# ufal/neuralmonkey

Measured on NVIDIA H100. Metric: train_target_tokens_per_sec, higher is better.
Workload: dtype f32 storage; tensor-core products in fp16 (vocabulary) / tf32 with fp32 accumulation

## Files before the change

neuralmonkey_b200/csrc/gru_cluster.cuh:

```cuda
#pragma once
#include "common.cuh"

namespace nm {

constexpr int GC_CLUSTER = 8;
constexpr int GC_SLICES = 32;
constexpr int GC_UPW = 4;
constexpr int GC_WARPS = 10;
constexpr int GC_THREADS = GC_WARPS * 32;
constexpr int GC_MAX_UNITS = GC_WARPS * GC_UPW;
constexpr int GC_RB = 2;
constexpr int GC_MAX_SL = 10;
constexpr int GC_SMEM_CAP = 200 * 1024;
constexpr int GC_BAR_BYTES = 64;
constexpr int GC_XS = 4;
constexpr int GC_PF = 8;

__host__ __device__ constexpr int gc_row(int SL) { return GC_SLICES * 4 * (((SL + 3) / 4) | 1); }
__host__ __device__ constexpr int gc_fwd_row_floats(int SL) {
  return 3 * gc_row(SL) + GC_MAX_UNITS * (1 + 2 * GC_XS) + 1;
}
__host__ __device__ constexpr int gc_bwd_row_floats(int SL) {
  return 4 * gc_row(SL) + GC_MAX_UNITS * (1 + 2 * GC_PF) + 1;
}

template <int SL>
struct GcGeom {
  static constexpr int SLP = 4 * (((SL + 3) / 4) | 1);
  static constexpr int ROW = GC_SLICES * SLP;
  static __device__ __forceinline__ int pos(int j) { return (j / SL) * SLP + (j % SL); }
};

__device__ __forceinline__ void cluster_barrier() {
  asm volatile("barrier.cluster.arrive.release.aligned;\n\tbarrier.cluster.wait.acquire.aligned;" ::
                   : "memory");
}
__device__ __forceinline__ uint32_t cluster_rank() {
  uint32_t r;
  asm volatile("mov.u32 %0, %%cluster_ctarank;" : "=r"(r));
  return r;
}

__device__ __forceinline__ uint32_t gc_smem_u32(const void* p) {
  return (uint32_t)__cvta_generic_to_shared(p);
}
__device__ __forceinline__ void gc_mbar_init(uint32_t bar) {
  asm volatile("mbarrier.init.shared::cta.b64 [%0], 1;" ::"r"(bar));
  asm volatile("fence.mbarrier_init.release.cluster;" ::: "memory");
}
__device__ __forceinline__ void gc_mbar_arm(uint32_t bar, uint32_t bytes) {
  asm volatile("mbarrier.arrive.expect_tx.shared::cta.b64 _, [%0], %1;" ::"r"(bar), "r"(bytes) : "memory");
}
__device__ __forceinline__ void gc_mbar_wait(uint32_t bar, uint32_t parity) {
  uint32_t done;
  do {
    asm volatile(
        "{\n\t.reg .pred p;\n\t"
        "mbarrier.try_wait.parity.acquire.cluster.shared::cta.b64 p, [%1], %2;\n\t"
        "selp.u32 %0, 1, 0, p;\n\t}"
        : "=r"(done)
        : "r"(bar), "r"(parity)
        : "memory");
  } while (!done);
}
__device__ __forceinline__ void gc_send(uint32_t addr, uint32_t bar, uint32_t dst, float v) {
  uint32_t ra, rb;
  asm volatile("mapa.shared::cluster.u32 %0, %1, %2;" : "=r"(ra) : "r"(addr), "r"(dst));
  asm volatile("mapa.shared::cluster.u32 %0, %1, %2;" : "=r"(rb) : "r"(bar), "r"(dst));
  asm volatile("st.async.shared::cluster.mbarrier::complete_tx::bytes.b32 [%0], %1, [%2];" ::"r"(ra),
               "r"(__float_as_uint(v)), "r"(rb)
               : "memory");
}

__device__ __forceinline__ void cp_async4(float* smem_dst, const float* gmem_src) {
  const uint32_t d = gc_smem_u32(smem_dst);
  asm volatile("cp.async.ca.shared.global [%0], [%1], 4;" ::"r"(d), "l"(gmem_src) : "memory");
}
__device__ __forceinline__ void cp_async_commit() { asm volatile("cp.async.commit_group;" ::: "memory"); }
__device__ __forceinline__ void cp_async_wait_all() { asm volatile("cp.async.wait_all;" ::: "memory"); }

template <int N, int O>
__device__ __forceinline__ void gc_reduce_level(float (&v)[N], int lane) {
  constexpr int n = N * O / 16;
  if constexpr (n > 1) {
    const bool upper = (lane & O) != 0;
#pragma unroll
    for (int i = 0; i < n / 2; ++i) {
      const float keep = upper ? v[i + n / 2] : v[i];
      const float send = upper ? v[i] : v[i + n / 2];
      v[i] = keep + __shfl_xor_sync(0xffffffffu, send, O);
    }
  } else {
    v[0] += __shfl_xor_sync(0xffffffffu, v[0], O);
  }
  if constexpr (O > 1) gc_reduce_level<N, O / 2>(v, lane);
}
template <int N>
__device__ __forceinline__ void gc_reduce_scatter(float (&v)[N], int lane) {
  gc_reduce_level<N, 16>(v, lane);
}

template <int SL>
__device__ __forceinline__ void gc_dot(const float* __restrict__ vec, int row0, int lane,
                                       const float (&w)[GC_UPW][SL], float (&acc)[GC_RB][GC_UPW]) {
#pragma unroll
  for (int r = 0; r < GC_RB; ++r)
#pragma unroll
    for (int u = 0; u < GC_UPW; ++u) acc[r][u] = 0.f;
  const float* base = vec + row0 * GcGeom<SL>::ROW + lane * GcGeom<SL>::SLP;
#pragma unroll
  for (int c = 0; c < SL; c += 4) {
    const int n = SL - c < 4 ? SL - c : 4;
#pragma unroll
    for (int r = 0; r < GC_RB; ++r) {
      const float* p = base + r * GcGeom<SL>::ROW + c;
      float x[4];
      if (n == 4) {
        const float4 q = *reinterpret_cast<const float4*>(p);
        x[0] = q.x; x[1] = q.y; x[2] = q.z; x[3] = q.w;
      } else {
        if (n >= 2) {
          const float2 q = *reinterpret_cast<const float2*>(p);
          x[0] = q.x; x[1] = q.y;
        }
        if (n == 1) x[0] = p[0];
        if (n == 3) x[2] = p[2];
      }
#pragma unroll
      for (int u = 0; u < GC_UPW; ++u)
#pragma unroll
        for (int i = 0; i < 4; ++i)
          if (i < n) acc[r][u] = fmaf(x[i], w[u][c + i], acc[r][u]);
    }
  }
}

template <int SL>
__device__ __forceinline__ void gc_load_w(float (&w)[GC_UPW][SL], const float* __restrict__ W,
                                          int64_t sk, int64_t su, int unit0, int unit_limit, int k0, int H) {
#pragma unroll
  for (int u = 0; u < GC_UPW; ++u)
#pragma unroll
    for (int i = 0; i < SL; ++i) {
      const int unit = unit0 + u, k = k0 + i;
      const bool ok = (unit < unit_limit) && (k < H);
      w[u][i] = ok ? W[(int64_t)k * sk + (int64_t)unit * su] : 0.f;
    }
}

struct GcProf {
  bool on;
  unsigned t0;
  __device__ __forceinline__ explicit GcProf(const long long* out)
      : on(out != nullptr && blockIdx.x == 0 && threadIdx.x == 0), t0(on ? (unsigned)clock() : 0u) {}
  __device__ __forceinline__ void lap(long long* out, int slot) {
    if (on) {
      const unsigned t1 = (unsigned)clock();
      out[slot] += (long long)(t1 - t0);
      t0 = t1;
    }
  }
};

struct GcFwdArgs {
  const float* xproj;
  const float* Wgh;
  const float* Wch;
  const float* h0;
  const int32_t* lengths;
  const float* drop_mask;
  float* states;
  float* raw_states;
  float* final_state;
  float* gates;
  float* hprev;
  float* rh;
  int B, T, H, Bc, reverse;
  long long* prof;
};

__device__ __forceinline__ void gc_fwd_prefetch(const GcFwdArgs& a, int t, float* dst, int b0, int nrows,
                                                int ubeg, int UW) {
  const int H = a.H, T = a.T;
  for (int idx = threadIdx.x; idx < a.Bc * UW; idx += GC_THREADS) {
    const int b = idx / UW, ul = idx - b * UW, j = ubeg + ul;
    if (b < nrows && j < H) {
      const int64_t row = ((int64_t)(b0 + b) * T + t);
      const float* xp = a.xproj + row * 3 * H + j;
      float* xd = dst + (b * GC_MAX_UNITS + ul) * GC_XS;
      cp_async4(xd, xp);
      cp_async4(xd + 1, xp + H);
      cp_async4(xd + 2, xp + 2 * H);
      if (a.drop_mask) cp_async4(xd + 3, a.drop_mask + row * H + j);
    }
  }
  cp_async_commit();
}

__device__ __forceinline__ uint32_t gc_phase_bytes(const GcFwdArgs& a) { return (uint32_t)(a.Bc * a.H * 4); }

template <int SL>
__global__ void __launch_bounds__(GC_THREADS, 1) gru_seq_fwd_cluster_kernel(GcFwdArgs a) {
  extern __shared__ __align__(16) float gc_smem[];
  constexpr int ROW = GcGeom<SL>::ROW;
  const int H = a.H, T = a.T, Bc = a.Bc;
  float* hbuf = gc_smem + GC_BAR_BYTES / 4;
  float* rhbuf = hbuf + 2 * Bc * ROW;
  float* us = rhbuf + Bc * ROW;
  float* xs = us + Bc * GC_MAX_UNITS;
  int* lens = reinterpret_cast<int*>(xs + 2 * Bc * GC_MAX_UNITS * GC_XS);
  const uint32_t bar_h = gc_smem_u32(gc_smem), bar_rh = bar_h + 16;

  const int rank = (int)cluster_rank();
  const int ubeg = rank * H / GC_CLUSTER;
  const int unit_limit = (rank + 1) * H / GC_CLUSTER;
  const int UW = unit_limit - ubeg;
  const int b0 = (blockIdx.x / GC_CLUSTER) * Bc;
  const int nrows = min(Bc, a.B - b0);
  const int lane = threadIdx.x & 31, warp = threadIdx.x >> 5;
  const int unit0_local = warp * GC_UPW;
  const int unit0 = ubeg + unit0_local;
  const bool warp_live = unit0 < unit_limit;

  float wr[GC_UPW][SL], wu[GC_UPW][SL], wc[GC_UPW][SL];
  gc_load_w<SL>(wr, a.Wgh, 2 * H, 1, unit0, unit_limit, lane * SL, H);
  gc_load_w<SL>(wu, a.Wgh + H, 2 * H, 1, unit0, unit_limit, lane * SL, H);
  gc_load_w<SL>(wc, a.Wch, H, 1, unit0, unit_limit, lane * SL, H);

  const int g1 = lane >> 4, r1 = (lane >> 3) & 1, u1 = (lane >> 1) & 3;
  const int r2 = (lane >> 4) & 1, u2 = (lane >> 2) & 3, copy2 = lane & 3;
  const int copy1 = ((lane >> 4) << 1) | (lane & 1);
  const bool ok1 = unit0 + u1 < unit_limit, ok2 = unit0 + u2 < unit_limit;
  const int j1 = unit0 + u1, j2 = unit0 + u2;
  const int pos1 = ok1 ? GcGeom<SL>::pos(j1) : 0, pos2 = ok2 ? GcGeom<SL>::pos(j2) : 0;

  if (threadIdx.x == 0) {
    gc_mbar_init(bar_h);
    gc_mbar_init(bar_h + 8);
    gc_mbar_init(bar_rh);
    gc_mbar_arm(bar_h, gc_phase_bytes(a));
    gc_mbar_arm(bar_h + 8, gc_phase_bytes(a));
    gc_mbar_arm(bar_rh, gc_phase_bytes(a));
  }
  for (int i = threadIdx.x; i < 3 * Bc * ROW; i += GC_THREADS) hbuf[i] = 0.f;
  for (int i = threadIdx.x; i < 2 * Bc * GC_MAX_UNITS * GC_XS; i += GC_THREADS) xs[i] = 0.f;
  for (int b = threadIdx.x; b < Bc; b += GC_THREADS)
    lens[b] = b < nrows ? (a.lengths ? a.lengths[b0 + b] : T) : 0;


  __syncthreads();
  cluster_barrier();
  const int t_first = a.reverse ? T - 1 : 0;
  for (int idx = threadIdx.x; idx < Bc * UW; idx += GC_THREADS) {
    const int b = idx / UW, j = ubeg + (idx - b * UW);
    const float hv = (b < nrows && a.h0) ? a.h0[(int64_t)(b0 + b) * H + j] : 0.f;
    if (b < nrows) a.hprev[((int64_t)(b0 + b) * T + t_first) * H + j] = hv;
    const uint32_t addr = gc_smem_u32(hbuf + b * ROW + GcGeom<SL>::pos(j));
    for (int d = 0; d < GC_CLUSTER; ++d) gc_send(addr, bar_h, d, hv);
  }
  gc_fwd_prefetch(a, t_first, xs, b0, nrows, ubeg, UW);

  GcProf prof(a.prof);
  for (int step = 0; step < T; ++step) {
    const int t = a.reverse ? T - 1 - step : step;
    const bool last = (step == T - 1);
    const int t_next = a.reverse ? t - 1 : t + 1;
    const int64_t row0 = (int64_t)b0 * T + t;
    const int par = step & 1;
    const float* hb = hbuf + par * Bc * ROW;
    const float* xc = xs + par * Bc * GC_MAX_UNITS * GC_XS;

    gc_mbar_wait(bar_h + 8 * par, (step >> 1) & 1);
    if (threadIdx.x == 0 && step + 2 < T) gc_mbar_arm(bar_h + 8 * par, gc_phase_bytes(a));
    prof.lap(a.prof, 0);
    cp_async_wait_all();
    __syncthreads();
    if (!last) gc_fwd_prefetch(a, t_next, xs + (par ^ 1) * Bc * GC_MAX_UNITS * GC_XS, b0, nrows, ubeg, UW);
    prof.lap(a.prof, 1);

    if (warp_live) {
      for (int r0 = 0; r0 < Bc; r0 += GC_RB) {
        float ar[GC_RB][GC_UPW], au[GC_RB][GC_UPW];
        gc_dot<SL>(hb, r0, lane, wr, ar);
        gc_dot<SL>(hb, r0, lane, wu, au);
        float v[2 * GC_RB * GC_UPW];
#pragma unroll
        for (int r = 0; r < GC_RB; ++r)
#pragma unroll
          for (int u = 0; u < GC_UPW; ++u) {
            v[r * GC_UPW + u] = ar[r][u];
            v[GC_RB * GC_UPW + r * GC_UPW + u] = au[r][u];
          }
        gc_reduce_scatter<2 * GC_RB * GC_UPW>(v, lane);
        const int b = r0 + r1, ul = unit0_local + u1;
        const float g = sigmoidf_(v[0] + xc[(b * GC_MAX_UNITS + ul) * GC_XS + g1]);
        const float rhv = g * hb[b * ROW + pos1];
        const float rh_peer = __shfl_xor_sync(0xffffffffu, rhv, 16);
        const float rh_send = g1 == 0 ? rhv : rh_peer;
        if (ok1) {
          if ((lane & 1) == 0) {
            if (b < nrows) {
              const int64_t row = row0 + (int64_t)b * T;
              a.gates[row * 3 * H + g1 * H + j1] = g;
              if (g1 == 0) a.rh[row * H + j1] = rhv;
            }
            if (g1 == 1) us[b * GC_MAX_UNITS + ul] = g;
          }
          const uint32_t addr = gc_smem_u32(rhbuf + b * ROW + pos1);
          gc_send(addr, bar_rh, 2 * copy1, rh_send);
          gc_send(addr, bar_rh, 2 * copy1 + 1, rh_send);
        }
      }
      __syncwarp();
    }
    prof.lap(a.prof, 2);
    gc_mbar_wait(bar_rh, step & 1);
    if (threadIdx.x == 0 && !last) gc_mbar_arm(bar_rh, gc_phase_bytes(a));
    prof.lap(a.prof, 3);

    if (warp_live) {
      const uint32_t bar_next = bar_h + 8 * (par ^ 1);
      float* hn_buf = hbuf + (par ^ 1) * Bc * ROW;
      for (int r0 = 0; r0 < Bc; r0 += GC_RB) {
        float ac[GC_RB][GC_UPW];
        gc_dot<SL>(rhbuf, r0, lane, wc, ac);
        float v[GC_RB * GC_UPW];
#pragma unroll
        for (int r = 0; r < GC_RB; ++r)
#pragma unroll
          for (int u = 0; u < GC_UPW; ++u) v[r * GC_UPW + u] = ac[r][u];
        gc_reduce_scatter<GC_RB * GC_UPW>(v, lane);
        if (!ok2) continue;
        const int b = r0 + r2, ul = unit0_local + u2;
        const float* xd = xc + (b * GC_MAX_UNITS + ul) * GC_XS;
        const float c = tanhf(v[0] + xd[2]);
        const float hv = hb[b * ROW + pos2];
        const float uu = us[b * GC_MAX_UNITS + ul];
        const bool live = t < lens[b];
        float hn = live ? (uu * hv + (1.f - uu) * c) : hv;
        const float raw = live ? hn : 0.f;
        if (a.drop_mask && live) hn *= xd[3];
        if (b < nrows) {
          const int64_t row = row0 + (int64_t)b * T;
          if (copy2 == 0) a.gates[row * 3 * H + 2 * H + j2] = c;
          else if (copy2 == 1) a.states[row * H + j2] = live ? hn : 0.f;
          else if (copy2 == 2) { if (a.raw_states) a.raw_states[row * H + j2] = raw; }
          else if (last) a.final_state[(int64_t)(b0 + b) * H + j2] = hn;
          else a.hprev[((int64_t)(b0 + b) * T + t_next) * H + j2] = hn;
        }
        if (!last) {
          const uint32_t addr = gc_smem_u32(hn_buf + b * ROW + pos2);
          gc_send(addr, bar_next, 2 * copy2, hn);
          gc_send(addr, bar_next, 2 * copy2 + 1, hn);
        }
      }
    }
    prof.lap(a.prof, 4);
  }
  cluster_barrier();
}

struct GcBwdArgs {
  const float* Wgh;
  const float* Wch;
  const int32_t* lengths;
  const float* drop_mask;
  const float* gates;
  const float* hprev;
  const float* dstates;
  const float* draw;
  const float* dfinal;
  float* dxproj;
  float* dh0;
  int B, T, H, Bc, reverse;
  long long* prof;
};

__device__ __forceinline__ float gc_bwd_e1(const GcBwdArgs& a, const float* pf, float dh, bool live,
                                           float& zc, float& zu) {
  if (!live) {
    zc = zu = 0.f;
    return dh;
  }
  const float uu = pf[1], c = pf[2], hv = pf[3];
  if (a.dstates) dh += pf[4];
  if (a.drop_mask) dh *= pf[5];
  if (a.draw) dh += pf[6];
  const float du = dh * (hv - c);
  const float dc = dh * (1.f - uu);
  zc = dc * (1.f - c * c);
  zu = du * uu * (1.f - uu);
  return dh * uu;
}

__device__ __forceinline__ void gc_bwd_prefetch(const GcBwdArgs& a, int t, float* dst, const int* lens, int b0,
                                                int ubeg, int UW) {
  const int H = a.H, T = a.T;
  for (int idx = threadIdx.x; idx < a.Bc * UW; idx += GC_THREADS) {
    const int b = idx / UW, u = idx - b * UW, j = ubeg + u;
    if (t >= lens[b]) continue;
    const int64_t row = (int64_t)(b0 + b) * T + t;
    float* d = dst + (b * GC_MAX_UNITS + u) * GC_PF;
    const float* g = a.gates + row * 3 * H + j;
    cp_async4(d, g);
    cp_async4(d + 1, g + H);
    cp_async4(d + 2, g + 2 * H);
    cp_async4(d + 3, a.hprev + row * H + j);
    if (a.dstates) cp_async4(d + 4, a.dstates + row * H + j);
    if (a.drop_mask) cp_async4(d + 5, a.drop_mask + row * H + j);
    if (a.draw) cp_async4(d + 6, a.draw + row * H + j);
  }
  cp_async_commit();
}

template <int SL>
__global__ void __launch_bounds__(GC_THREADS, 1) gru_seq_bwd_cluster_kernel(GcBwdArgs a) {
  extern __shared__ __align__(16) float gc_smem[];
  constexpr int ROW = GcGeom<SL>::ROW;
  const int H = a.H, T = a.T, Bc = a.Bc;
  float* vc = gc_smem + GC_BAR_BYTES / 4;
  float* vu = vc + Bc * ROW;
  float* vr = vu + 2 * Bc * ROW;
  float* dhp = vr + Bc * ROW;
  float* pf = dhp + Bc * GC_MAX_UNITS;
  int* lens = reinterpret_cast<int*>(pf + 2 * Bc * GC_MAX_UNITS * GC_PF);
  const uint32_t bar_a = gc_smem_u32(gc_smem), bar_b = bar_a + 16;
  const uint32_t bytes_a = (uint32_t)(2 * Bc * H * 4), bytes_b = (uint32_t)(Bc * H * 4);

  const int rank = (int)cluster_rank();
  const int ubeg = rank * H / GC_CLUSTER;
  const int unit_limit = (rank + 1) * H / GC_CLUSTER;
  const int UW = unit_limit - ubeg;
  const int b0 = (blockIdx.x / GC_CLUSTER) * Bc;
  const int nrows = min(Bc, a.B - b0);
  const int lane = threadIdx.x & 31, warp = threadIdx.x >> 5;
  const int unit0_local = warp * GC_UPW;
  const int unit0 = ubeg + unit0_local;
  const bool warp_live = unit0 < unit_limit;

  float w1[GC_UPW][SL], w2r[GC_UPW][SL], w2u[GC_UPW][SL];
  gc_load_w<SL>(w1, a.Wch, 1, H, unit0, unit_limit, lane * SL, H);
  gc_load_w<SL>(w2r, a.Wgh, 1, 2 * H, unit0, unit_limit, lane * SL, H);
  gc_load_w<SL>(w2u, a.Wgh + H, 1, 2 * H, unit0, unit_limit, lane * SL, H);

  const int rr_ = (lane >> 4) & 1, uq = (lane >> 2) & 3, copy = lane & 3;
  const bool ok = unit0 + uq < unit_limit;
  const int ji = unit0 + uq, ul = unit0_local + uq;
  const int pos = ok ? GcGeom<SL>::pos(ji) : 0;
  auto time_of = [reverse = a.reverse, T](int k) { return reverse ? k : T - 1 - k; };

  if (threadIdx.x == 0) {
    gc_mbar_init(bar_a);
    gc_mbar_init(bar_a + 8);
    gc_mbar_init(bar_b);
    gc_mbar_arm(bar_a, bytes_a);
    gc_mbar_arm(bar_a + 8, bytes_a);
    gc_mbar_arm(bar_b, bytes_b);
  }
  for (int i = threadIdx.x; i < 4 * Bc * ROW; i += GC_THREADS) vc[i] = 0.f;
  for (int i = threadIdx.x; i < 2 * Bc * GC_MAX_UNITS * GC_PF; i += GC_THREADS) pf[i] = 0.f;
  for (int b = threadIdx.x; b < Bc; b += GC_THREADS)
    lens[b] = b < nrows ? (a.lengths ? a.lengths[b0 + b] : T) : 0;
  __syncthreads();


  gc_bwd_prefetch(a, time_of(0), pf, lens, b0, ubeg, UW);
  cp_async_wait_all();
  __syncthreads();
  cluster_barrier();
  {
    const int t = time_of(0);
    for (int idx = threadIdx.x; idx < Bc * UW; idx += GC_THREADS) {
      const int b = idx / UW, u = idx - b * UW, j = ubeg + u;
      const bool live = t < lens[b];
      const float dh = (a.dfinal && b < nrows) ? a.dfinal[(int64_t)(b0 + b) * H + j] : 0.f;
      float zc, zu;
      dhp[b * GC_MAX_UNITS + u] = gc_bwd_e1(a, pf + (b * GC_MAX_UNITS + u) * GC_PF, dh, live, zc, zu);
      if (b < nrows) {
        const int64_t row = (int64_t)(b0 + b) * T + t;
        a.dxproj[row * 3 * H + H + j] = zu;
        a.dxproj[row * 3 * H + 2 * H + j] = zc;
      }
      const int p = GcGeom<SL>::pos(j);
      const uint32_t ac = gc_smem_u32(vc + b * ROW + p), au = gc_smem_u32(vu + b * ROW + p);
      for (int d = 0; d < GC_CLUSTER; ++d) {
        gc_send(ac, bar_a, d, zc);
        gc_send(au, bar_a, d, zu);
      }
    }
  }

  GcProf prof(a.prof);
  for (int k = 0; k < T; ++k) {
    const int t = time_of(k);
    const bool last = (k == T - 1);
    const int64_t row0 = (int64_t)b0 * T + t;
    const int par = k & 1;
    const float* pfc = pf + par * Bc * GC_MAX_UNITS * GC_PF;
    float* pfn = pf + (par ^ 1) * Bc * GC_MAX_UNITS * GC_PF;

    gc_mbar_wait(bar_a + 8 * par, (k >> 1) & 1);
    if (threadIdx.x == 0 && k + 2 < T) gc_mbar_arm(bar_a + 8 * par, bytes_a);
    prof.lap(a.prof, 0);
    __syncthreads();
    if (!last) gc_bwd_prefetch(a, time_of(k + 1), pfn, lens, b0, ubeg, UW);
    prof.lap(a.prof, 1);

    if (warp_live) {
      for (int r0 = 0; r0 < Bc; r0 += GC_RB) {
        float acc[GC_RB][GC_UPW];
        gc_dot<SL>(vc, r0, lane, w1, acc);
        float v[GC_RB * GC_UPW];
#pragma unroll
        for (int r = 0; r < GC_RB; ++r)
#pragma unroll
          for (int u = 0; u < GC_UPW; ++u) v[r * GC_UPW + u] = acc[r][u];
        gc_reduce_scatter<GC_RB * GC_UPW>(v, lane);
        if (!ok) continue;
        const int b = r0 + rr_;
        const float drh = v[0];
        const bool live = t < lens[b];
        const float* s = pfc + (b * GC_MAX_UNITS + ul) * GC_PF;
        const float rg = s[0], hv = s[3];
        const float zr = live ? drh * hv * rg * (1.f - rg) : 0.f;
        if (copy == 0) {
          if (b < nrows) a.dxproj[(row0 + (int64_t)b * T) * 3 * H + ji] = zr;
          if (live) dhp[b * GC_MAX_UNITS + ul] += drh * rg;
        }
        const uint32_t addr = gc_smem_u32(vr + b * ROW + pos);
        gc_send(addr, bar_b, 2 * copy, zr);
        gc_send(addr, bar_b, 2 * copy + 1, zr);
      }
      __syncwarp();
    }
    prof.lap(a.prof, 2);
    gc_mbar_wait(bar_b, k & 1);
    if (threadIdx.x == 0 && !last) gc_mbar_arm(bar_b, bytes_b);
    prof.lap(a.prof, 3);
    cp_async_wait_all();
    __syncthreads();
    prof.lap(a.prof, 4);

    if (warp_live) {
      const float* vuc = vu + par * Bc * ROW;
      const int tn = last ? t : time_of(k + 1);
      for (int r0 = 0; r0 < Bc; r0 += GC_RB) {
        float accr[GC_RB][GC_UPW], accu[GC_RB][GC_UPW];
        gc_dot<SL>(vr, r0, lane, w2r, accr);
        gc_dot<SL>(vuc, r0, lane, w2u, accu);
        float v[GC_RB * GC_UPW];
#pragma unroll
        for (int r = 0; r < GC_RB; ++r)
#pragma unroll
          for (int u = 0; u < GC_UPW; ++u) v[r * GC_UPW + u] = accr[r][u] + accu[r][u];
        gc_reduce_scatter<GC_RB * GC_UPW>(v, lane);
        const int b = r0 + rr_;
        const float dcarry = ok ? dhp[b * GC_MAX_UNITS + ul] + v[0] : 0.f;
        __syncwarp();
        if (!ok) continue;
        if (last) {
          if (a.dh0 && copy == 0 && b < nrows) a.dh0[(int64_t)(b0 + b) * H + ji] = dcarry;
          continue;
        }
        float zc, zu;
        const float d = gc_bwd_e1(a, pfn + (b * GC_MAX_UNITS + ul) * GC_PF, dcarry, tn < lens[b], zc, zu);
        if (b < nrows) {
          const int64_t row = (int64_t)(b0 + b) * T + tn;
          if (copy == 1) a.dxproj[row * 3 * H + H + ji] = zu;
          else if (copy == 2) a.dxproj[row * 3 * H + 2 * H + ji] = zc;
        }
        if (copy == 0) dhp[b * GC_MAX_UNITS + ul] = d;
        const uint32_t ac = gc_smem_u32(vc + b * ROW + pos);
        const uint32_t au = gc_smem_u32(vu + ((par ^ 1) * Bc + b) * ROW + pos);
        const uint32_t bar_next = bar_a + 8 * (par ^ 1);
        gc_send(ac, bar_next, 2 * copy, zc);
        gc_send(ac, bar_next, 2 * copy + 1, zc);
        gc_send(au, bar_next, 2 * copy, zu);
        gc_send(au, bar_next, 2 * copy + 1, zu);
      }
    }
    prof.lap(a.prof, 5);
  }
  cluster_barrier();
}

}
```

Baseline: 1.259 million.

## Batch cluster DSMEM exchanges into 16-byte vector stores with per-rank quad layout

```diff
diff --git a/neuralmonkey_b200/csrc/gru_cluster.cuh b/neuralmonkey_b200/csrc/gru_cluster.cuh
--- a/neuralmonkey_b200/csrc/gru_cluster.cuh
+++ b/neuralmonkey_b200/csrc/gru_cluster.cuh
@@ -26,9 +26,13 @@
 
 template <int SL>
 struct GcGeom {
-  static constexpr int SLP = 4 * (((SL + 3) / 4) | 1);
-  static constexpr int ROW = GC_SLICES * SLP;
-  static __device__ __forceinline__ int pos(int j) { return (j / SL) * SLP + (j % SL); }
+  static constexpr int UP = 4 * SL;
+  static constexpr int ROW = gc_row(SL);
+  static constexpr int V = SL % 4 == 0 ? 4 : SL % 2 == 0 ? 2 : 1;
+  static __device__ __forceinline__ int slice_pos(int lane, int e) {
+    const int swz = SL == 8 ? ((lane >> 2) & 1) * 4 : 0;
+    return lane * SL + (e ^ swz);
+  }
 };
 
 __device__ __forceinline__ void cluster_barrier() {
@@ -71,6 +75,37 @@
                "r"(__float_as_uint(v)), "r"(rb)
                : "memory");
 }
+__device__ __forceinline__ void gc_send4(uint32_t addr, uint32_t bar, uint32_t dst, const float (&v)[4]) {
+  uint32_t ra, rb;
+  asm volatile("mapa.shared::cluster.u32 %0, %1, %2;" : "=r"(ra) : "r"(addr), "r"(dst));
+  asm volatile("mapa.shared::cluster.u32 %0, %1, %2;" : "=r"(rb) : "r"(bar), "r"(dst));
+  asm volatile("st.async.shared::cluster.mbarrier::complete_tx::bytes.v4.b32 [%0], {%1, %2, %3, %4}, [%5];" ::
+                   "r"(ra), "r"(__float_as_uint(v[0])), "r"(__float_as_uint(v[1])), "r"(__float_as_uint(v[2])),
+               "r"(__float_as_uint(v[3])), "r"(rb)
+               : "memory");
+}
+template <int KEEP, int SRC>
+__device__ __forceinline__ float gc_shfl_keep(float x) {
+  uint32_t o;
+  asm volatile("shfl.sync.idx.b32 %0, %1, %2, %3, 0xffffffff;"
+               : "=r"(o)
+               : "r"(__float_as_uint(x)), "n"(SRC), "n"((KEEP << 8) | 0x1f));
+  return __uint_as_float(o);
+}
+template <int KEEP, int STRIDE>
+__device__ __forceinline__ void gc_gather4(float (&q)[4], float x) {
+  static_assert((KEEP & (3 * STRIDE)) == 0, "the unit bits of the source lane come from STRIDE * u");
+  q[0] = gc_shfl_keep<KEEP, 0>(x);
+  q[1] = gc_shfl_keep<KEEP, STRIDE>(x);
+  q[2] = gc_shfl_keep<KEEP, 2 * STRIDE>(x);
+  q[3] = gc_shfl_keep<KEEP, 3 * STRIDE>(x);
+}
+__device__ __forceinline__ uint32_t gc_quad_bytes(int H, int Bc) {
+  int quads = 0;
+#pragma unroll
+  for (int r = 0; r < GC_CLUSTER; ++r) quads += ((r + 1) * H / GC_CLUSTER - r * H / GC_CLUSTER + 3) / 4;
+  return (uint32_t)(Bc * 16 * quads);
+}
 
 __device__ __forceinline__ void cp_async4(float* smem_dst, const float* gmem_src) {
   const uint32_t d = gc_smem_u32(smem_dst);
@@ -82,7 +117,7 @@
 template <int N, int O>
 __device__ __forceinline__ void gc_reduce_level(float (&v)[N], int lane) {
   constexpr int n = N * O / 16;
-  if constexpr (n > 1) {
+  if constexpr (n == 2 * GC_UPW) {
     const bool upper = (lane & O) != 0;
 #pragma unroll
     for (int i = 0; i < n / 2; ++i) {
@@ -90,6 +125,9 @@
       const float send = upper ? v[i] : v[i + n / 2];
       v[i] = keep + __shfl_xor_sync(0xffffffffu, send, O);
     }
+  } else if constexpr (n > 1) {
+#pragma unroll
+    for (int i = 0; i < n / 2; ++i) v[i] += __shfl_xor_sync(0xffffffffu, v[i + n / 2], O);
   } else {
     v[0] += __shfl_xor_sync(0xffffffffu, v[0], O);
   }
@@ -97,55 +135,58 @@
 }
 template <int N>
 __device__ __forceinline__ void gc_reduce_scatter(float (&v)[N], int lane) {
+  static_assert(N == GC_RB * GC_UPW || N == 2 * GC_RB * GC_UPW, "gate, row and unit index bits");
   gc_reduce_level<N, 16>(v, lane);
 }
 
 template <int SL>
 __device__ __forceinline__ void gc_dot(const float* __restrict__ vec, int row0, int lane,
                                        const float (&w)[GC_UPW][SL], float (&acc)[GC_RB][GC_UPW]) {
+  constexpr int V = GcGeom<SL>::V;
 #pragma unroll
   for (int r = 0; r < GC_RB; ++r)
 #pragma unroll
     for (int u = 0; u < GC_UPW; ++u) acc[r][u] = 0.f;
-  const float* base = vec + row0 * GcGeom<SL>::ROW + lane * GcGeom<SL>::SLP;
-#pragma unroll
-  for (int c = 0; c < SL; c += 4) {
-    const int n = SL - c < 4 ? SL - c : 4;
+  const float* base = vec + row0 * GcGeom<SL>::ROW;
+#pragma unroll
+  for (int c = 0; c < SL; c += V) {
 #pragma unroll
     for (int r = 0; r < GC_RB; ++r) {
-      const float* p = base + r * GcGeom<SL>::ROW + c;
-      float x[4];
-      if (n == 4) {
+      const float* p = base + r * GcGeom<SL>::ROW + GcGeom<SL>::slice_pos(lane, c);
+      float x[V];
+      if constexpr (V == 4) {
         const float4 q = *reinterpret_cast<const float4*>(p);
         x[0] = q.x; x[1] = q.y; x[2] = q.z; x[3] = q.w;
+      } else if constexpr (V == 2) {
+        const float2 q = *reinterpret_cast<const float2*>(p);
+        x[0] = q.x; x[1] = q.y;
       } else {
-        if (n >= 2) {
-          const float2 q = *reinterpret_cast<const float2*>(p);
-          x[0] = q.x; x[1] = q.y;
-        }
-        if (n == 1) x[0] = p[0];
-        if (n == 3) x[2] = p[2];
+        x[0] = p[0];
       }
 #pragma unroll
       for (int u = 0; u < GC_UPW; ++u)
 #pragma unroll
-        for (int i = 0; i < 4; ++i)
-          if (i < n) acc[r][u] = fmaf(x[i], w[u][c + i], acc[r][u]);
+        for (int i = 0; i < V; ++i) acc[r][u] = fmaf(x[i], w[u][c + i], acc[r][u]);
     }
   }
 }
 
 template <int SL>
 __device__ __forceinline__ void gc_load_w(float (&w)[GC_UPW][SL], const float* __restrict__ W,
-                                          int64_t sk, int64_t su, int unit0, int unit_limit, int k0, int H) {
-#pragma unroll
-  for (int u = 0; u < GC_UPW; ++u)
-#pragma unroll
-    for (int i = 0; i < SL; ++i) {
-      const int unit = unit0 + u, k = k0 + i;
-      const bool ok = (unit < unit_limit) && (k < H);
-      w[u][i] = ok ? W[(int64_t)k * sk + (int64_t)unit * su] : 0.f;
-    }
+                                          int64_t sk, int64_t su, int unit0, int usw, int unit_limit, int lane,
+                                          int H) {
+  const int r = lane >> 2;
+  const int k0 = r * H / GC_CLUSTER - r * GcGeom<SL>::UP, k_end = (r + 1) * H / GC_CLUSTER;
+#pragma unroll
+  for (int e = 0; e < SL; ++e) {
+    const int k = k0 + GcGeom<SL>::slice_pos(lane, e);
+    const bool k_ok = k < k_end;
+#pragma unroll
+    for (int u = 0; u < GC_UPW; ++u) {
+      const int unit = unit0 + (u ^ usw);
+      w[u][e] = (k_ok && unit < unit_limit) ? W[(int64_t)k * sk + (int64_t)unit * su] : 0.f;
+    }
+  }
 }
 
 struct GcProf {
@@ -197,8 +238,6 @@
   cp_async_commit();
 }
 
-__device__ __forceinline__ uint32_t gc_phase_bytes(const GcFwdArgs& a) { return (uint32_t)(a.Bc * a.H * 4); }
-
 template <int SL>
 __global__ void __launch_bounds__(GC_THREADS, 1) gru_seq_fwd_cluster_kernel(GcFwdArgs a) {
   extern __shared__ __align__(16) float gc_smem[];
@@ -222,25 +261,23 @@
   const int unit0 = ubeg + unit0_local;
   const bool warp_live = unit0 < unit_limit;
 
-  float wr[GC_UPW][SL], wu[GC_UPW][SL], wc[GC_UPW][SL];
-  gc_load_w<SL>(wr, a.Wgh, 2 * H, 1, unit0, unit_limit, lane * SL, H);
-  gc_load_w<SL>(wu, a.Wgh + H, 2 * H, 1, unit0, unit_limit, lane * SL, H);
-  gc_load_w<SL>(wc, a.Wch, H, 1, unit0, unit_limit, lane * SL, H);
-
   const int g1 = lane >> 4, r1 = (lane >> 3) & 1, u1 = (lane >> 1) & 3;
   const int r2 = (lane >> 4) & 1, u2 = (lane >> 2) & 3, copy2 = lane & 3;
-  const int copy1 = ((lane >> 4) << 1) | (lane & 1);
+  float wg[2][GC_UPW][SL], wc[GC_UPW][SL];
+  gc_load_w<SL>(wg[0], a.Wgh + g1 * H, 2 * H, 1, unit0, u1, unit_limit, lane, H);
+  gc_load_w<SL>(wg[1], a.Wgh + (g1 ^ 1) * H, 2 * H, 1, unit0, u1, unit_limit, lane, H);
+  gc_load_w<SL>(wc, a.Wch, H, 1, unit0, u2, unit_limit, lane, H);
   const bool ok1 = unit0 + u1 < unit_limit, ok2 = unit0 + u2 < unit_limit;
   const int j1 = unit0 + u1, j2 = unit0 + u2;
-  const int pos1 = ok1 ? GcGeom<SL>::pos(j1) : 0, pos2 = ok2 ? GcGeom<SL>::pos(j2) : 0;
+  const int pos1 = rank * GcGeom<SL>::UP + unit0_local + u1, pos2 = rank * GcGeom<SL>::UP + unit0_local + u2;
 
   if (threadIdx.x == 0) {
     gc_mbar_init(bar_h);
     gc_mbar_init(bar_h + 8);
     gc_mbar_init(bar_rh);
-    gc_mbar_arm(bar_h, gc_phase_bytes(a));
-    gc_mbar_arm(bar_h + 8, gc_phase_bytes(a));
-    gc_mbar_arm(bar_rh, gc_phase_bytes(a));
+    gc_mbar_arm(bar_h, (uint32_t)(Bc * H * 4));
+    gc_mbar_arm(bar_h + 8, gc_quad_bytes(H, Bc));
+    gc_mbar_arm(bar_rh, gc_quad_bytes(H, Bc));
   }
   for (int i = threadIdx.x; i < 3 * Bc * ROW; i += GC_THREADS) hbuf[i] = 0.f;
   for (int i = threadIdx.x; i < 2 * Bc * GC_MAX_UNITS * GC_XS; i += GC_THREADS) xs[i] = 0.f;
@@ -252,10 +289,10 @@
   cluster_barrier();
   const int t_first = a.reverse ? T - 1 : 0;
   for (int idx = threadIdx.x; idx < Bc * UW; idx += GC_THREADS) {
-    const int b = idx / UW, j = ubeg + (idx - b * UW);
+    const int b = idx / UW, ul = idx - b * UW, j = ubeg + ul;
     const float hv = (b < nrows && a.h0) ? a.h0[(int64_t)(b0 + b) * H + j] : 0.f;
     if (b < nrows) a.hprev[((int64_t)(b0 + b) * T + t_first) * H + j] = hv;
-    const uint32_t addr = gc_smem_u32(hbuf + b * ROW + GcGeom<SL>::pos(j));
+    const uint32_t addr = gc_smem_u32(hbuf + b * ROW + rank * GcGeom<SL>::UP + ul);
     for (int d = 0; d < GC_CLUSTER; ++d) gc_send(addr, bar_h, d, hv);
   }
   gc_fwd_prefetch(a, t_first, xs, b0, nrows, ubeg, UW);
@@ -271,7 +308,7 @@
     const float* xc = xs + par * Bc * GC_MAX_UNITS * GC_XS;
 
     gc_mbar_wait(bar_h + 8 * par, (step >> 1) & 1);
-    if (threadIdx.x == 0 && step + 2 < T) gc_mbar_arm(bar_h + 8 * par, gc_phase_bytes(a));
+    if (threadIdx.x == 0 && step + 2 < T) gc_mbar_arm(bar_h + 8 * par, gc_quad_bytes(H, Bc));
     prof.lap(a.prof, 0);
     cp_async_wait_all();
     __syncthreads();
@@ -280,47 +317,58 @@
 
     if (warp_live) {
       for (int r0 = 0; r0 < Bc; r0 += GC_RB) {
-        float ar[GC_RB][GC_UPW], au[GC_RB][GC_UPW];
-        gc_dot<SL>(hb, r0, lane, wr, ar);
-        gc_dot<SL>(hb, r0, lane, wu, au);
+        float a0[GC_RB][GC_UPW], a1[GC_RB][GC_UPW];
+        gc_dot<SL>(hb, r0, lane, wg[0], a0);
+        gc_dot<SL>(hb, r0, lane, wg[1], a1);
         float v[2 * GC_RB * GC_UPW];
 #pragma unroll
         for (int r = 0; r < GC_RB; ++r)
 #pragma unroll
           for (int u = 0; u < GC_UPW; ++u) {
-            v[r * GC_UPW + u] = ar[r][u];
-            v[GC_RB * GC_UPW + r * GC_UPW + u] = au[r][u];
+            v[r * GC_UPW + u] = a0[r][u];
+            v[GC_RB * GC_UPW + r * GC_UPW + u] = a1[r][u];
           }
         gc_reduce_scatter<2 * GC_RB * GC_UPW>(v, lane);
         const int b = r0 + r1, ul = unit0_local + u1;
         const float g = sigmoidf_(v[0] + xc[(b * GC_MAX_UNITS + ul) * GC_XS + g1]);
-        const float rhv = g * hb[b * ROW + pos1];
-        const float rh_peer = __shfl_xor_sync(0xffffffffu, rhv, 16);
-        const float rh_send = g1 == 0 ? rhv : rh_peer;
-        if (ok1) {
-          if ((lane & 1) == 0) {
-            if (b < nrows) {
-              const int64_t row = row0 + (int64_t)b * T;
-              a.gates[row * 3 * H + g1 * H + j1] = g;
-              if (g1 == 0) a.rh[row * H + j1] = rhv;
-            }
-            if (g1 == 1) us[b * GC_MAX_UNITS + ul] = g;
+        const float rhv = ok1 ? g * hb[b * ROW + pos1] : 0.f;
+        float q[4];
+        gc_gather4<0x18, 2>(q, rhv);
+        if (lane < 16) gc_send4(gc_smem_u32(rhbuf + b * ROW + (pos1 & ~3)), bar_rh, lane & 7, q);
+        if (ok1 && (lane & 1) == 0) {
+          if (b < nrows) {
+            const int64_t row = row0 + (int64_t)b * T;
+            a.gates[row * 3 * H + g1 * H + j1] = g;
+            if (g1 == 0) a.rh[row * H + j1] = rhv;
           }
-          const uint32_t addr = gc_smem_u32(rhbuf + b * ROW + pos1);
-          gc_send(addr, bar_rh, 2 * copy1, rh_send);
-          gc_send(addr, bar_rh, 2 * copy1 + 1, rh_send);
+          if (g1 == 1) us[b * GC_MAX_UNITS + ul] = g;
         }
       }
       __syncwarp();
     }
     prof.lap(a.prof, 2);
     gc_mbar_wait(bar_rh, step & 1);
-    if (threadIdx.x == 0 && !last) gc_mbar_arm(bar_rh, gc_phase_bytes(a));
+    if (threadIdx.x == 0 && !last) gc_mbar_arm(bar_rh, gc_quad_bytes(H, Bc));
     prof.lap(a.prof, 3);
 
     if (warp_live) {
       const uint32_t bar_next = bar_h + 8 * (par ^ 1);
       float* hn_buf = hbuf + (par ^ 1) * Bc * ROW;
+      float* out;
+      int64_t out_step = (int64_t)T * H;
+      if (copy2 == 0) {
+        out = a.gates + row0 * 3 * H + 2 * H + j2;
+        out_step = (int64_t)T * 3 * H;
+      } else if (copy2 == 1) {
+        out = a.states + row0 * H + j2;
+      } else if (copy2 == 2) {
+        out = a.raw_states ? a.raw_states + row0 * H + j2 : nullptr;
+      } else if (last) {
+        out = a.final_state + (int64_t)b0 * H + j2;
+        out_step = H;
+      } else {
+        out = a.hprev + ((int64_t)b0 * T + t_next) * H + j2;
+      }
       for (int r0 = 0; r0 < Bc; r0 += GC_RB) {
         float ac[GC_RB][GC_UPW];
         gc_dot<SL>(rhbuf, r0, lane, wc, ac);
@@ -330,7 +378,6 @@
 #pragma unroll
           for (int u = 0; u < GC_UPW; ++u) v[r * GC_UPW + u] = ac[r][u];
         gc_reduce_scatter<GC_RB * GC_UPW>(v, lane);
-        if (!ok2) continue;
         const int b = r0 + r2, ul = unit0_local + u2;
         const float* xd = xc + (b * GC_MAX_UNITS + ul) * GC_XS;
         const float c = tanhf(v[0] + xd[2]);
@@ -340,18 +387,14 @@
         float hn = live ? (uu * hv + (1.f - uu) * c) : hv;
         const float raw = live ? hn : 0.f;
         if (a.drop_mask && live) hn *= xd[3];
-        if (b < nrows) {
-          const int64_t row = row0 + (int64_t)b * T;
-          if (copy2 == 0) a.gates[row * 3 * H + 2 * H + j2] = c;
-          else if (copy2 == 1) a.states[row * H + j2] = live ? hn : 0.f;
-          else if (copy2 == 2) { if (a.raw_states) a.raw_states[row * H + j2] = raw; }
-          else if (last) a.final_state[(int64_t)(b0 + b) * H + j2] = hn;
-          else a.hprev[((int64_t)(b0 + b) * T + t_next) * H + j2] = hn;
+        if (!last) {
+          float q[4];
+          gc_gather4<0x10, 4>(q, ok2 ? hn : 0.f);
+          if ((lane & 8) == 0) gc_send4(gc_smem_u32(hn_buf + b * ROW + (pos2 & ~3)), bar_next, lane & 7, q);
         }
-        if (!last) {
-          const uint32_t addr = gc_smem_u32(hn_buf + b * ROW + pos2);
-          gc_send(addr, bar_next, 2 * copy2, hn);
-          gc_send(addr, bar_next, 2 * copy2 + 1, hn);
+        if (ok2 && b < nrows && out) {
+          const float val = copy2 == 0 ? c : copy2 == 1 ? (live ? hn : 0.f) : copy2 == 2 ? raw : hn;
+          out[b * out_step] = val;
         }
       }
     }
@@ -425,7 +468,6 @@
   float* pf = dhp + Bc * GC_MAX_UNITS;
   int* lens = reinterpret_cast<int*>(pf + 2 * Bc * GC_MAX_UNITS * GC_PF);
   const uint32_t bar_a = gc_smem_u32(gc_smem), bar_b = bar_a + 16;
-  const uint32_t bytes_a = (uint32_t)(2 * Bc * H * 4), bytes_b = (uint32_t)(Bc * H * 4);
 
   const int rank = (int)cluster_rank();
   const int ubeg = rank * H / GC_CLUSTER;
@@ -438,24 +480,23 @@
   const int unit0 = ubeg + unit0_local;
   const bool warp_live = unit0 < unit_limit;
 
+  const int rr_ = (lane >> 4) & 1, uq = (lane >> 2) & 3, copy = lane & 3;
   float w1[GC_UPW][SL], w2r[GC_UPW][SL], w2u[GC_UPW][SL];
-  gc_load_w<SL>(w1, a.Wch, 1, H, unit0, unit_limit, lane * SL, H);
-  gc_load_w<SL>(w2r, a.Wgh, 1, 2 * H, unit0, unit_limit, lane * SL, H);
-  gc_load_w<SL>(w2u, a.Wgh + H, 1, 2 * H, unit0, unit_limit, lane * SL, H);
-
-  const int rr_ = (lane >> 4) & 1, uq = (lane >> 2) & 3, copy = lane & 3;
+  gc_load_w<SL>(w1, a.Wch, 1, H, unit0, uq, unit_limit, lane, H);
+  gc_load_w<SL>(w2r, a.Wgh, 1, 2 * H, unit0, uq, unit_limit, lane, H);
+  gc_load_w<SL>(w2u, a.Wgh + H, 1, 2 * H, unit0, uq, unit_limit, lane, H);
   const bool ok = unit0 + uq < unit_limit;
   const int ji = unit0 + uq, ul = unit0_local + uq;
-  const int pos = ok ? GcGeom<SL>::pos(ji) : 0;
+  const int quad = rank * GcGeom<SL>::UP + unit0_local;
   auto time_of = [reverse = a.reverse, T](int k) { return reverse ? k : T - 1 - k; };
 
   if (threadIdx.x == 0) {
     gc_mbar_init(bar_a);
     gc_mbar_init(bar_a + 8);
     gc_mbar_init(bar_b);
-    gc_mbar_arm(bar_a, bytes_a);
-    gc_mbar_arm(bar_a + 8, bytes_a);
-    gc_mbar_arm(bar_b, bytes_b);
+    gc_mbar_arm(bar_a, (uint32_t)(2 * Bc * H * 4));
+    gc_mbar_arm(bar_a + 8, 2 * gc_quad_bytes(H, Bc));
+    gc_mbar_arm(bar_b, gc_quad_bytes(H, Bc));
   }
   for (int i = threadIdx.x; i < 4 * Bc * ROW; i += GC_THREADS) vc[i] = 0.f;
   for (int i = threadIdx.x; i < 2 * Bc * GC_MAX_UNITS * GC_PF; i += GC_THREADS) pf[i] = 0.f;
@@ -481,7 +522,7 @@
         a.dxproj[row * 3 * H + H + j] = zu;
         a.dxproj[row * 3 * H + 2 * H + j] = zc;
       }
-      const int p = GcGeom<SL>::pos(j);
+      const int p = rank * GcGeom<SL>::UP + u;
       const uint32_t ac = gc_smem_u32(vc + b * ROW + p), au = gc_smem_u32(vu + b * ROW + p);
       for (int d = 0; d < GC_CLUSTER; ++d) {
         gc_send(ac, bar_a, d, zc);
@@ -500,7 +541,7 @@
     float* pfn = pf + (par ^ 1) * Bc * GC_MAX_UNITS * GC_PF;
 
     gc_mbar_wait(bar_a + 8 * par, (k >> 1) & 1);
-    if (threadIdx.x == 0 && k + 2 < T) gc_mbar_arm(bar_a + 8 * par, bytes_a);
+    if (threadIdx.x == 0 && k + 2 < T) gc_mbar_arm(bar_a + 8 * par, 2 * gc_quad_bytes(H, Bc));
     prof.lap(a.prof, 0);
     __syncthreads();
     if (!last) gc_bwd_prefetch(a, time_of(k + 1), pfn, lens, b0, ubeg, UW);
@@ -516,26 +557,25 @@
 #pragma unroll
           for (int u = 0; u < GC_UPW; ++u) v[r * GC_UPW + u] = acc[r][u];
         gc_reduce_scatter<GC_RB * GC_UPW>(v, lane);
-        if (!ok) continue;
         const int b = r0 + rr_;
         const float drh = v[0];
         const bool live = t < lens[b];
         const float* s = pfc + (b * GC_MAX_UNITS + ul) * GC_PF;
         const float rg = s[0], hv = s[3];
-        const float zr = live ? drh * hv * rg * (1.f - rg) : 0.f;
-        if (copy == 0) {
+        const float zr = (ok && live) ? drh * hv * rg * (1.f - rg) : 0.f;
+        if (ok && copy == 0) {
           if (b < nrows) a.dxproj[(row0 + (int64_t)b * T) * 3 * H + ji] = zr;
           if (live) dhp[b * GC_MAX_UNITS + ul] += drh * rg;
         }
-        const uint32_t addr = gc_smem_u32(vr + b * ROW + pos);
-        gc_send(addr, bar_b, 2 * copy, zr);
-        gc_send(addr, bar_b, 2 * copy + 1, zr);
+        float q[4];
+        gc_gather4<0x10, 4>(q, zr);
+        if ((lane & 8) == 0) gc_send4(gc_smem_u32(vr + b * ROW + quad), bar_b, lane & 7, q);
       }
       __syncwarp();
     }
     prof.lap(a.prof, 2);
     gc_mbar_wait(bar_b, k & 1);
-    if (threadIdx.x == 0 && !last) gc_mbar_arm(bar_b, bytes_b);
+    if (threadIdx.x == 0 && !last) gc_mbar_arm(bar_b, gc_quad_bytes(H, Bc));
     prof.lap(a.prof, 3);
     cp_async_wait_all();
     __syncthreads();
@@ -543,6 +583,7 @@
 
     if (warp_live) {
       const float* vuc = vu + par * Bc * ROW;
+      float* const send_buf = (lane & 2) ? vu + (par ^ 1) * Bc * ROW : vc;
       const int tn = last ? t : time_of(k + 1);
       for (int r0 = 0; r0 < Bc; r0 += GC_RB) {
         float accr[GC_RB][GC_UPW], accu[GC_RB][GC_UPW];
@@ -557,26 +598,23 @@
         const int b = r0 + rr_;
         const float dcarry = ok ? dhp[b * GC_MAX_UNITS + ul] + v[0] : 0.f;
         __syncwarp();
-        if (!ok) continue;
         if (last) {
-          if (a.dh0 && copy == 0 && b < nrows) a.dh0[(int64_t)(b0 + b) * H + ji] = dcarry;
+          if (ok && a.dh0 && copy == 0 && b < nrows) a.dh0[(int64_t)(b0 + b) * H + ji] = dcarry;
           continue;
         }
         float zc, zu;
         const float d = gc_bwd_e1(a, pfn + (b * GC_MAX_UNITS + ul) * GC_PF, dcarry, tn < lens[b], zc, zu);
-        if (b < nrows) {
-          const int64_t row = (int64_t)(b0 + b) * T + tn;
-          if (copy == 1) a.dxproj[row * 3 * H + H + ji] = zu;
-          else if (copy == 2) a.dxproj[row * 3 * H + 2 * H + ji] = zc;
+        if (ok) {
+          if (b < nrows) {
+            const int64_t row = (int64_t)(b0 + b) * T + tn;
+            if (copy == 1) a.dxproj[row * 3 * H + H + ji] = zu;
+            else if (copy == 2) a.dxproj[row * 3 * H + 2 * H + ji] = zc;
+          }
+          if (copy == 0) dhp[b * GC_MAX_UNITS + ul] = d;
         }
-        if (copy == 0) dhp[b * GC_MAX_UNITS + ul] = d;
-        const uint32_t ac = gc_smem_u32(vc + b * ROW + pos);
-        const uint32_t au = gc_smem_u32(vu + ((par ^ 1) * Bc + b) * ROW + pos);
-        const uint32_t bar_next = bar_a + 8 * (par ^ 1);
-        gc_send(ac, bar_next, 2 * copy, zc);
-        gc_send(ac, bar_next, 2 * copy + 1, zc);
-        gc_send(au, bar_next, 2 * copy, zu);
-        gc_send(au, bar_next, 2 * copy + 1, zu);
+        float q[4];
+        gc_gather4<0x12, 4>(q, ok ? (copy & 2 ? zu : zc) : 0.f);
+        gc_send4(gc_smem_u32(send_buf + b * ROW + quad), bar_a + 8 * (par ^ 1), ((lane >> 1) & 6) | (lane & 1), q);
       }
     }
     prof.lap(a.prof, 5);
```

Measured after the change: 1.310 million (median of 6 runs). +4.0%, better.
